# enoche/MMRec

Measured on NVIDIA H100. Metric: graph-prop edges/sec (+ full-catalog scored-items/sec in extra) @ d=64, higher is better.
Workload: dtype f32

## Files before the change

mmrec_b200/csrc/project_tc.cu:

```cuda
#include "tc_common.cuh"

namespace mmrec {

using namespace tc;

constexpr int PJ_M = 128;
constexpr int PJ_KC = 32;
constexpr int PJ_LBO_A = 2064;
constexpr int PJ_A_BYTES = (PJ_KC / 4) * PJ_LBO_A;
constexpr int PJ_CONV = 256;
constexpr int PJ_THREADS = PJ_CONV + 32;
template <int N> constexpr int pj_depth() { return N == 64 ? 3 : (N == 128 ? 2 : 1); }

struct ProjParams {
    const float* table; int64_t F; const int64_t* idx; int64_t n_out;
    const float *Whi, *Wlo;
    int N, n_chunks, chunks_per_split, n_splits, stages, vec_ok, n_tiles;
    float* partial;
    int64_t rows_padded;
};

struct PjSmem {
    uint32_t a0, b0, bars, total, stage_bytes, b_bytes;
};
__host__ __device__ inline PjSmem pj_smem(int N, int stages) {
    PjSmem L;
    L.b_bytes = (uint32_t)N * PJ_KC * 4;
    L.stage_bytes = 2 * PJ_A_BYTES + 2 * L.b_bytes;
    L.a0 = 0;
    L.b0 = 2 * PJ_A_BYTES;
    L.bars = stages * L.stage_bytes;
    L.total = L.bars + 32 * 8;
    return L;
}

template <int N, bool FAST>
__global__ void __launch_bounds__(PJ_THREADS, 1) project_tc_kernel(const ProjParams p) {
    constexpr int PJ_DEPTH = pj_depth<N>();
    extern __shared__ __align__(1024) uint8_t smem[];
    const PjSmem L = pj_smem(N, p.stages);
    const uint32_t sbase = smem_u32(smem);
    const uint32_t bar = sbase + L.bars;
    const int warp = threadIdx.x >> 5, lane = threadIdx.x & 31;
    if (threadIdx.x == 0) {
        for (int s = 0; s < 8; ++s) { mbar_init(bar + s * 8, PJ_CONV); mbar_init(bar + (8 + s) * 8, 1); mbar_init(bar + (16 + s) * 8, PJ_CONV / 32); }
        mbar_fence_init();
    }
    __syncthreads();

    const int tile = blockIdx.x / p.n_splits, sp = blockIdx.x % p.n_splits;
    const int c0 = sp * p.chunks_per_split;
    const int c1 = min(p.n_chunks, c0 + p.chunks_per_split);
    const int n_my = c1 - c0;
    const int rot = n_my > 0 ? ((int)(((int64_t)tile * n_my) / p.n_tiles) / PJ_DEPTH * PJ_DEPTH) % n_my : 0;

    if (warp == PJ_CONV / 32) {
        if (lane == 0) {
            int s = 0;
            uint32_t par = 1;
            for (int c = 0; c < n_my; ++c) {
                mbar_wait(bar + (16 + s) * 8, par);
                mbar_expect_tx(bar + (8 + s) * 8, 2 * L.b_bytes);
                const int64_t off = (int64_t)(c0 + (c + rot) % n_my) * (L.b_bytes / 4);
                bulk_g2s(sbase + s * L.stage_bytes + L.b0, p.Whi + off, L.b_bytes, bar + (8 + s) * 8);
                bulk_g2s(sbase + s * L.stage_bytes + L.b0 + L.b_bytes, p.Wlo + off, L.b_bytes, bar + (8 + s) * 8);
                if (++s == p.stages) { s = 0; par ^= 1; }
            }
        }
        return;
    }
    const int t = threadIdx.x;
    const int g = t >> 7;
    const int kb = t & 7;
    const float* rowp[4];
#pragma unroll
    for (int i = 0; i < 4; ++i) {
        const int64_t r = (int64_t)tile * PJ_M + (t >> 3) + 32 * i;
        rowp[i] = r < p.n_out ? p.table + (p.idx ? p.idx[r] : r) * p.F : nullptr;
    }
    int ld_c = rot;
    const float* kp[4];
#pragma unroll
    for (int i = 0; i < 4; ++i) kp[i] = rowp[i] ? rowp[i] + (int64_t)c0 * PJ_KC + kb * 4 : nullptr;
    auto load_chunk = [&](int c, float4 (&x)[4]) {
        if (FAST) {
            const bool on = c < n_my;
#pragma unroll
            for (int i = 0; i < 4; ++i)
                x[i] = (on && kp[i]) ? __ldg(reinterpret_cast<const float4*>(kp[i] + ld_c * PJ_KC)) : make_float4(0.f, 0.f, 0.f, 0.f);
            if (on && ++ld_c == n_my) ld_c = 0;
            return;
        }
        const int64_t k = (int64_t)(c0 + (c + rot) % n_my) * PJ_KC + kb * 4;
#pragma unroll
        for (int i = 0; i < 4; ++i) {
            float4 v = make_float4(0.f, 0.f, 0.f, 0.f);
            if (rowp[i] && c < n_my) {
                if (p.vec_ok && k + 3 < p.F) v = __ldg(reinterpret_cast<const float4*>(rowp[i] + k));
                else {
                    if (k + 0 < p.F) v.x = __ldg(rowp[i] + k + 0);
                    if (k + 1 < p.F) v.y = __ldg(rowp[i] + k + 1);
                    if (k + 2 < p.F) v.z = __ldg(rowp[i] + k + 2);
                    if (k + 3 < p.F) v.w = __ldg(rowp[i] + k + 3);
                }
            }
            x[i] = v;
        }
    };
    const uint32_t LBO_B = (uint32_t)(N / 8) * 128;
    const uint64_t a_hi0 = smem_desc(sbase + L.a0 + g * 1024, PJ_LBO_A, 128), a_lo0 = smem_desc(sbase + L.a0 + PJ_A_BYTES + g * 1024, PJ_LBO_A, 128);
    const uint64_t b_hi0 = smem_desc(sbase + L.b0, LBO_B, 128), b_lo0 = smem_desc(sbase + L.b0 + L.b_bytes, LBO_B, 128);
    const uint64_t ka = (2 * PJ_LBO_A) >> 4, kbs = (2 * LBO_B) >> 4;
    float acc[N / 2];
#pragma unroll
    for (int i = 0; i < N / 2; ++i) acc[i] = 0.f;
    uint32_t first = 0;
    int prev = 0;
    float4 ringA[PJ_DEPTH][4], ringB[PJ_DEPTH][4];
    int s = 0;
    uint32_t par = 1;
    int done = 0;
    auto fill = [&](int cbase, float4 (&ring)[PJ_DEPTH][4]) {
#pragma unroll
        for (int q = 0; q < PJ_DEPTH; ++q) load_chunk(cbase + q, ring[q]);
    };
    auto drain = [&](int cbase, float4 (&ring)[PJ_DEPTH][4]) {
#pragma unroll
        for (int q = 0; q < PJ_DEPTH; ++q) {
            if (cbase + q < n_my) {
                mbar_wait(bar + (16 + s) * 8, par);
                uint8_t* st = smem + s * L.stage_bytes;
#pragma unroll
                for (int i = 0; i < 4; ++i) {
                    const int r = (t >> 3) + 32 * i;
                    const uint32_t off = kb * PJ_LBO_A + (r >> 3) * 128 + (r & 7) * 16;
                    float4 h, l;
                    split_tf32_trunc(ring[q][i].x, h.x, l.x); split_tf32_trunc(ring[q][i].y, h.y, l.y);
                    split_tf32_trunc(ring[q][i].z, h.z, l.z); split_tf32_trunc(ring[q][i].w, h.w, l.w);
                    *reinterpret_cast<float4*>(st + L.a0 + off) = h;
                    *reinterpret_cast<float4*>(st + L.a0 + PJ_A_BYTES + off) = l;
                }
                fence_proxy_async();
                mbar_arrive(bar + s * 8);
                mbar_wait(bar + s * 8, par ^ 1);
                mbar_wait(bar + (8 + s) * 8, par ^ 1);
                const uint64_t st_off = (uint64_t)(s * L.stage_bytes) >> 4;
                uint64_t a_hi = a_hi0 + st_off, a_lo = a_lo0 + st_off, b_hi = b_hi0 + st_off, b_lo = b_lo0 + st_off;
                wgmma_fence();
#pragma unroll
                for (int j = 0; j < PJ_KC / 8; ++j) {
                    wgmma_tf32<N>(acc, a_hi, b_hi, first);
                    first = 1;
                    wgmma_tf32<N>(acc, a_lo, b_hi, 1);
                    wgmma_tf32<N>(acc, a_hi, b_lo, 1);
                    a_hi += ka; a_lo += ka; b_hi += kbs; b_lo += kbs;
                }
                wgmma_commit();
                if (done++ > 0) {
                    wgmma_wait<1>();
                    warp_arrive(bar + (16 + prev) * 8);
                }
                prev = s;
                if (++s == p.stages) { s = 0; par ^= 1; }
            }
        }
    };
    fill(0, ringA);
    for (int cb = 0; cb < n_my; cb += 2 * PJ_DEPTH) {
        fill(cb + PJ_DEPTH, ringB);
        drain(cb, ringA);
        fill(cb + 2 * PJ_DEPTH, ringA);
        drain(cb + PJ_DEPTH, ringB);
    }
    wgmma_wait<0>();
    wgmma_fence_regs(acc);
    const int w = (t >> 5) & 3;
    const int64_t row0 = (int64_t)tile * PJ_M + g * 64 + w * 16 + (lane >> 2);
#pragma unroll
    for (int h = 0; h < 2; ++h) {
        float* dst = p.partial + ((int64_t)sp * p.rows_padded + row0 + 8 * h) * N + 2 * (lane & 3);
#pragma unroll
        for (int j = 0; j < N / 8; ++j)
            *reinterpret_cast<float2*>(dst + 8 * j) = make_float2(acc[4 * j + 2 * h], acc[4 * j + 2 * h + 1]);
    }
}

__global__ void __launch_bounds__(256) project_reduce_kernel(int64_t n_out, int d, int N, int n_splits, int64_t rows_padded,
                                                             const float* __restrict__ partial, const float* __restrict__ bias,
                                                             int l2, float* __restrict__ Y, int64_t ldy) {
    const int lane = threadIdx.x & 31;
    const int64_t row = (int64_t)blockIdx.x * 8 + (threadIdx.x >> 5);
    if (row >= n_out) return;
    float acc[8];
    float ss = 0.f;
#pragma unroll
    for (int i = 0; i < 8; ++i) {
        const int c = lane + 32 * i;
        float a = 0.f;
        if (c < d) {
            for (int s = 0; s < n_splits; ++s) a += partial[((int64_t)s * rows_padded + row) * N + c];
            if (bias) a += __ldg(bias + c);
            ss += a * a;
        }
        acc[i] = a;
    }
    float inv = 1.f;
    if (l2) { ss = warp_sum(ss); inv = 1.0f / fmaxf(sqrtf(ss), 1e-12f); }
#pragma unroll
    for (int i = 0; i < 8; ++i) {
        const int c = lane + 32 * i;
        if (c < d) Y[row * ldy + c] = l2 ? acc[i] * inv : acc[i];
    }
}

struct PjPlan {
    int N, KP, n_chunks, n_splits, chunks_per_split, stages;
    int64_t n_tiles, rows_padded;
    size_t off_whi, off_wlo, off_partial, total;
};

static bool pj_plan(int64_t n_out, int64_t F, int d, PjPlan& P) {
    if (d > 256 || n_out <= 0 || F < 1) return false;
    P.N = d <= 64 ? 64 : (d <= 128 ? 128 : 256);
    P.KP = (int)((F + PJ_KC - 1) / PJ_KC * PJ_KC);
    P.n_chunks = P.KP / PJ_KC;
    P.n_tiles = (n_out + PJ_M - 1) / PJ_M;
    P.rows_padded = P.n_tiles * PJ_M;
    const int sms = sm_count();
    int splits = (int)(sms / P.n_tiles);
    if (splits < 1) splits = 1;
    if (splits > P.n_chunks / 4) splits = P.n_chunks / 4 > 0 ? P.n_chunks / 4 : 1;
    if (splits > 32) splits = 32;
    P.chunks_per_split = (P.n_chunks + splits - 1) / splits;
    P.n_splits = (P.n_chunks + P.chunks_per_split - 1) / P.chunks_per_split;
    const uint32_t stage = 2 * PJ_A_BYTES + 2 * (uint32_t)P.N * PJ_KC * 4;
    P.stages = (int)((220 * 1024) / stage);
    if (P.stages > 8) P.stages = 8;
    if (P.stages < 2) return false;
    size_t off = 0;
    auto take = [&](size_t bytes) { size_t o = off; off += align_up(bytes, 1024); return o; };
    P.off_whi = take((size_t)P.N * P.KP * 4);
    P.off_wlo = take((size_t)P.N * P.KP * 4);
    P.off_partial = take((size_t)P.n_splits * P.rows_padded * P.N * 4);
    P.total = off + 1024;
    return true;
}

size_t project_tc_workspace_bytes(int64_t n_out, int64_t F, int d) {
    PjPlan P;
    return pj_plan(n_out, F, d, P) ? P.total : 0;
}

template <int R>
static int pack_weights(const float* W, int64_t F, int d, int KP, float* hi, float* lo, cudaStream_t stream) {
    const int64_t total = (int64_t)R * (KP / 4);
    pack_split_kernel<R><<<(unsigned)((total + 255) / 256), 256, 0, stream>>>(d, nullptr, W, F, (int)F, KP, hi, lo, 1);
    MMREC_LAUNCH_CHECK();
    return MMREC_OK;
}

int project_tc(int64_t n_out, const int64_t* idx, const float* table, int64_t F, const float* W, const float* bias, int d,
               int l2_normalize, float* Y, int64_t ldy, void* ws, size_t ws_bytes, cudaStream_t stream) {
    PjPlan P;
    if (!ws || !pj_plan(n_out, F, d, P) || ws_bytes < P.total || F >= (1ll << 31)) return 0;
    char* base = (char*)(((uintptr_t)ws + 1023) & ~(uintptr_t)1023);
    float *Whi = (float*)(base + P.off_whi), *Wlo = (float*)(base + P.off_wlo), *partial = (float*)(base + P.off_partial);
    int rc = P.N == 64 ? pack_weights<64>(W, F, d, P.KP, Whi, Wlo, stream)
                       : (P.N == 128 ? pack_weights<128>(W, F, d, P.KP, Whi, Wlo, stream) : pack_weights<256>(W, F, d, P.KP, Whi, Wlo, stream));
    if (rc) return rc;
    ProjParams p;
    p.table = table; p.F = F; p.idx = idx; p.n_out = n_out; p.Whi = Whi; p.Wlo = Wlo; p.N = P.N; p.n_chunks = P.n_chunks;
    p.chunks_per_split = P.chunks_per_split; p.n_splits = P.n_splits; p.stages = P.stages;
    p.n_tiles = (int)P.n_tiles;
    p.vec_ok = ((F & 3) == 0) && ((((uintptr_t)table) & 15) == 0);
    p.partial = partial; p.rows_padded = P.rows_padded;
    const PjSmem L = pj_smem(P.N, P.stages);
    rc = set_smem_once<project_tc_kernel<64, true>, project_tc_kernel<64, false>, project_tc_kernel<128, true>,
                       project_tc_kernel<128, false>, project_tc_kernel<256, true>, project_tc_kernel<256, false>>(227 * 1024);
    if (rc) return rc;
    const bool fast = p.vec_ok && (F % PJ_KC) == 0;
    const unsigned grid = (unsigned)(P.n_tiles * P.n_splits);
    if (P.N == 64) {
        if (fast) project_tc_kernel<64, true><<<grid, PJ_THREADS, L.total, stream>>>(p);
        else project_tc_kernel<64, false><<<grid, PJ_THREADS, L.total, stream>>>(p);
    } else if (P.N == 128) {
        if (fast) project_tc_kernel<128, true><<<grid, PJ_THREADS, L.total, stream>>>(p);
        else project_tc_kernel<128, false><<<grid, PJ_THREADS, L.total, stream>>>(p);
    } else {
        if (fast) project_tc_kernel<256, true><<<grid, PJ_THREADS, L.total, stream>>>(p);
        else project_tc_kernel<256, false><<<grid, PJ_THREADS, L.total, stream>>>(p);
    }
    MMREC_LAUNCH_CHECK();
    project_reduce_kernel<<<(unsigned)((n_out + 7) / 8), 256, 0, stream>>>(n_out, d, P.N, P.n_splits, P.rows_padded, partial, bias,
                                                                         l2_normalize, Y, ldy);
    MMREC_LAUNCH_CHECK();
    return 1;
}

}
```

mmrec_b200/csrc/spmm.cu:

```cuda
#include <cooperative_groups.h>

#include "common.cuh"

namespace mmrec {

struct SpmmParams {
    int64_t n_rows, n_cols;
    const int32_t* rowptr; const int32_t* colidx; const float* vals;
    const int4* tasks; int64_t n_tasks, n_heavy; const int4* split_rows; int32_t* counters; float* partial;
    const float* X; int64_t ldx;
    float* Y; int64_t ldy;
    const float* acc_in; float* acc_out; int64_t ldacc; float acc_div;
    const float* gate_ref; int64_t ldgate;
    int y_acc;
    const float* post; int64_t post_row0; uint32_t spost;
    int d;
    uint32_t sx, sy, sacc, sgate;
    const float* X_hi; const float* acc_in_hi;
    int x_split, acc_split;
    uint32_t sx_hi, sacc_hi;
};


__device__ __forceinline__ const float4* row_f4(const float* base, uint32_t stride, int r, int f4) {
    return reinterpret_cast<const float4*>(reinterpret_cast<const char*>(base) + (uint64_t)(uint32_t)r * stride) + f4;
}
__device__ __forceinline__ float4* row_f4(float* base, uint32_t stride, int r, int f4) {
    return reinterpret_cast<float4*>(reinterpret_cast<char*>(base) + (uint64_t)(uint32_t)r * stride) + f4;
}

template <bool TWO>
__device__ __forceinline__ float4 acc_in_f4(const SpmmParams& p, int r, int f4) {
    const bool hi = TWO && r >= p.acc_split;
    return *row_f4(hi ? p.acc_in_hi : p.acc_in, hi ? p.sacc_hi : p.sacc, hi ? r - p.acc_split : r, f4);
}

template <int D, int T>
struct VecCfg {
    static_assert(D % (4 * T) == 0, "row must split into float4 per lane");
    static constexpr int V = D / (4 * T);
    static constexpr int GPW = 32 / T;
    static constexpr int UNR = (V >= 4) ? 2 : (V == 2 ? 4 : 8);
};

template <int D, int T>
__device__ __forceinline__ void spmm_epilogue(const SpmmParams& p, bool on, int row, int l, float4 (&y)[VecCfg<D, T>::V],
                                              const float4 (&accin)[VecCfg<D, T>::V]) {
    using C = VecCfg<D, T>;
    if (p.gate_ref) {
        float dot = 0.f, ny = 0.f, nr = 0.f;
        if (on) {
#pragma unroll
            for (int v = 0; v < C::V; ++v) {
                float4 r = __ldg(row_f4(p.gate_ref, p.sgate, row, v * T + l));
                dot += y[v].x * r.x + y[v].y * r.y + y[v].z * r.z + y[v].w * r.w;
                ny += y[v].x * y[v].x + y[v].y * y[v].y + y[v].z * y[v].z + y[v].w * y[v].w;
                nr += r.x * r.x + r.y * r.y + r.z * r.z + r.w * r.w;
            }
        }
#pragma unroll
        for (int o = T / 2; o > 0; o >>= 1) {
            dot += __shfl_xor_sync(0xffffffffu, dot, o);
            ny += __shfl_xor_sync(0xffffffffu, ny, o);
            nr += __shfl_xor_sync(0xffffffffu, nr, o);
        }
        float c = dot / (fmaxf(sqrtf(ny), 1e-8f) * fmaxf(sqrtf(nr), 1e-8f));
#pragma unroll
        for (int v = 0; v < C::V; ++v) { y[v].x *= c; y[v].y *= c; y[v].z *= c; y[v].w *= c; }
    }
    if (!on) return;
    if (p.Y) {
#pragma unroll
        for (int v = 0; v < C::V; ++v) {
            float4 o = y[v];
            if (p.y_acc) {
                const float4 q = *row_f4(p.Y, p.sy, row, v * T + l);
                o.x += q.x; o.y += q.y; o.z += q.z; o.w += q.w;
            }
            *row_f4(p.Y, p.sy, row, v * T + l) = o;
        }
    }
    if (p.acc_out) {
#pragma unroll
        for (int v = 0; v < C::V; ++v) {
            float4 a = y[v];
            if (p.acc_in) { a.x += accin[v].x; a.y += accin[v].y; a.z += accin[v].z; a.w += accin[v].w; }
            if (p.acc_div != 1.0f) {
                a.x = __fdiv_rn(a.x, p.acc_div); a.y = __fdiv_rn(a.y, p.acc_div);
                a.z = __fdiv_rn(a.z, p.acc_div); a.w = __fdiv_rn(a.w, p.acc_div);
            }
            if (p.post && row >= p.post_row0) {
                const float4 q = *row_f4(p.post, p.spost, row - (int)p.post_row0, v * T + l);
                a.x += q.x; a.y += q.y; a.z += q.z; a.w += q.w;
            }
            *row_f4(p.acc_out, p.sacc, row, v * T + l) = a;
        }
    }
}

template <int D, int T, bool TWO>
__device__ __forceinline__ void spmm_gather(const SpmmParams& p, int b, int len, int maxlen, int l, float4 (&acc)[VecCfg<D, T>::V]) {
    using C = VecCfg<D, T>;
    int cj[C::UNR]; float wj[C::UNR];
    const int32_t* cp = p.colidx + b;
    const float* vp = p.vals + b;
    const float* xl = p.X + l * 4;
    const float* xh = TWO ? p.X_hi + l * 4 : xl;
#pragma unroll
    for (int u = 0; u < C::UNR; ++u) {
        const bool ok = u < len;
        cj[u] = ok ? __ldg(cp + u) : 0;
        wj[u] = ok ? __ldg(vp + u) : 0.f;
    }
    for (int j0 = 0; j0 < maxlen; j0 += C::UNR, cp += C::UNR, vp += C::UNR) {
        float4 x[C::UNR][C::V];
#pragma unroll
        for (int u = 0; u < C::UNR; ++u) {
            const bool ok = j0 + u < len;
            const bool hi = TWO && cj[u] >= p.x_split;
            const float* xb = hi ? xh : xl;
            const uint32_t sb = hi ? p.sx_hi : p.sx;
            const int rb = hi ? cj[u] - p.x_split : cj[u];
#pragma unroll
            for (int v = 0; v < C::V; ++v)
                x[u][v] = ok ? __ldg(row_f4(xb, sb, rb, v * T)) : make_float4(0.f, 0.f, 0.f, 0.f);
        }
        float wc[C::UNR];
#pragma unroll
        for (int u = 0; u < C::UNR; ++u) wc[u] = wj[u];
#pragma unroll
        for (int u = 0; u < C::UNR; ++u) {
            const bool ok = j0 + C::UNR + u < len;
            cj[u] = ok ? __ldg(cp + C::UNR + u) : 0;
            wj[u] = ok ? __ldg(vp + C::UNR + u) : 0.f;
        }
#pragma unroll
        for (int u = 0; u < C::UNR; ++u) {
#pragma unroll
            for (int v = 0; v < C::V; ++v) {
                acc[v].x = fmaf(wc[u], x[u][v].x, acc[v].x);
                acc[v].y = fmaf(wc[u], x[u][v].y, acc[v].y);
                acc[v].z = fmaf(wc[u], x[u][v].z, acc[v].z);
                acc[v].w = fmaf(wc[u], x[u][v].w, acc[v].w);
            }
        }
    }
}

template <int D, int T, bool TWO>
__device__ __forceinline__ bool spmm_split_finish(const SpmmParams& p, bool split, int row, int b, int sid, int l,
                                                  float4 (&acc)[VecCfg<D, T>::V], float4 (&accin)[VecCfg<D, T>::V]) {
    using C = VecCfg<D, T>;
    int4 sr = make_int4(0, 1, 0, 1);
    int old = -1;
    bool last = false;
    if (split) {
        sr = __ldg(p.split_rows + sid);
        const int seg = (b - sr.z) / sr.w;
        float* slot = p.partial + ((int64_t)sr.x + seg) * D;
#pragma unroll
        for (int v = 0; v < C::V; ++v) *reinterpret_cast<float4*>(slot + (v * T + l) * 4) = acc[v];
        __threadfence();
    }
    __syncwarp();
    if (split && l == 0) old = atomicAdd(p.counters + sid, 1);
    old = __shfl_sync(0xffffffffu, old, 0, T);
    if (split && old == sr.y - 1) {
        __threadfence();
#pragma unroll
        for (int v = 0; v < C::V; ++v) acc[v] = make_float4(0.f, 0.f, 0.f, 0.f);
        constexpr int RB = 8;
        for (int s2 = 0; s2 < sr.y; s2 += RB) {
            float4 q[RB][C::V];
#pragma unroll
            for (int r = 0; r < RB; ++r) {
                const float* ps = p.partial + ((int64_t)sr.x + s2 + r) * D;
#pragma unroll
                for (int v = 0; v < C::V; ++v)
                    q[r][v] = (s2 + r < sr.y) ? __ldcg(reinterpret_cast<const float4*>(ps + (v * T + l) * 4))
                                              : make_float4(0.f, 0.f, 0.f, 0.f);
            }
#pragma unroll
            for (int r = 0; r < RB; ++r) {
#pragma unroll
                for (int v = 0; v < C::V; ++v) {
                    acc[v].x += q[r][v].x; acc[v].y += q[r][v].y; acc[v].z += q[r][v].z; acc[v].w += q[r][v].w;
                }
            }
        }
        if (p.acc_in) {
#pragma unroll
            for (int v = 0; v < C::V; ++v)
                accin[v] = acc_in_f4<TWO>(p, row, v * T + l);
        }
        if (l == 0) p.counters[sid] = 0;
        last = true;
    }
    __syncwarp();
    return last;
}

template <int D, int T, bool TWO>
__device__ __forceinline__ void spmm_vec_body(const SpmmParams& p, float* __restrict__ red) {
    using C = VecCfg<D, T>;
    constexpr int G = 256 / T;
    const int lane = threadIdx.x & 31, warp = threadIdx.x >> 5;
    const int g = lane / T, l = lane % T;
    const int64_t n_work = p.tasks ? p.n_tasks : p.n_rows;
    const int64_t n_heavy = p.tasks ? p.n_heavy : 0;

    for (int64_t ct = blockIdx.x; ct < n_heavy; ct += gridDim.x) {
        const int4 tk = __ldg(p.tasks + ct);
        const int row = tk.x, sid = tk.w;
        const int len = tk.z - tk.y;
        const int chunk = (len + G - 1) / G;
        const int gi = warp * C::GPW + g;
        const int mb = tk.y + gi * chunk;
        int mylen = tk.z - mb;
        mylen = mylen < 0 ? 0 : (mylen > chunk ? chunk : mylen);
        float4 accin[C::V];
#pragma unroll
        for (int v = 0; v < C::V; ++v) accin[v] = make_float4(0.f, 0.f, 0.f, 0.f);
        if (warp == 0 && g == 0 && p.acc_in && sid < 0) {
#pragma unroll
            for (int v = 0; v < C::V; ++v)
                accin[v] = acc_in_f4<TWO>(p, row, v * T + l);
        }
        float4 acc[C::V];
#pragma unroll
        for (int v = 0; v < C::V; ++v) acc[v] = make_float4(0.f, 0.f, 0.f, 0.f);
        spmm_gather<D, T, TWO>(p, mb, mylen, chunk, l, acc);
#pragma unroll
        for (int v = 0; v < C::V; ++v) *reinterpret_cast<float4*>(red + gi * D + (v * T + l) * 4) = acc[v];
        __syncthreads();
        if (warp == 0) {
#pragma unroll
            for (int v = 0; v < C::V; ++v) acc[v] = make_float4(0.f, 0.f, 0.f, 0.f);
            if (g == 0) {
                for (int q = 0; q < G; ++q) {
#pragma unroll
                    for (int v = 0; v < C::V; ++v) {
                        const float4 r4 = *reinterpret_cast<const float4*>(red + q * D + (v * T + l) * 4);
                        acc[v].x += r4.x; acc[v].y += r4.y; acc[v].z += r4.z; acc[v].w += r4.w;
                    }
                }
            }
            bool do_epi = g == 0 && sid < 0;
            if (sid >= 0) do_epi = spmm_split_finish<D, T, TWO>(p, g == 0, row, tk.y, sid, l, acc, accin);
            spmm_epilogue<D, T>(p, do_epi, row, l, acc, accin);
        }
        __syncthreads();
    }

    const int64_t W = (int64_t)gridDim.x * (blockDim.x >> 5);
    const int64_t w = (int64_t)blockIdx.x * (blockDim.x >> 5) + warp;
    const int64_t n_light = n_work - n_heavy;
    auto slot_of = [&](int64_t it) -> int64_t { return it * W + ((it & 1) ? (W - 1 - w) : w); };
    auto fetch = [&](int64_t slot) -> int4 {
        const int64_t t = slot * C::GPW + g;
        if (t >= n_light) return make_int4(-1, 0, 0, -1);
        if (p.tasks) return __ldg(p.tasks + n_heavy + t);
        return make_int4((int)t, __ldg(p.rowptr + t), __ldg(p.rowptr + t + 1), -1);
    };
    const int64_t n_slots = (n_light + C::GPW - 1) / C::GPW;
    const int64_t n_iter = (n_slots + W - 1) / W;
    int4 nxt = fetch(slot_of(0));
    for (int64_t it = 0; it < n_iter; ++it) {
        const int row = nxt.x, b = nxt.y, sid = nxt.w;
        const int len = nxt.z - nxt.y;
        const bool valid = row >= 0;
        nxt = fetch(slot_of(it + 1));
        const int maxlen = __reduce_max_sync(0xffffffffu, valid ? len : 0);
        float4 accin[C::V];
#pragma unroll
        for (int v = 0; v < C::V; ++v) accin[v] = make_float4(0.f, 0.f, 0.f, 0.f);
        if (valid && p.acc_in && sid < 0) {
#pragma unroll
            for (int v = 0; v < C::V; ++v)
                accin[v] = acc_in_f4<TWO>(p, row, v * T + l);
        }
        float4 acc[C::V];
#pragma unroll
        for (int v = 0; v < C::V; ++v) acc[v] = make_float4(0.f, 0.f, 0.f, 0.f);
        spmm_gather<D, T, TWO>(p, b, valid ? len : 0, maxlen, l, acc);
        bool do_epi = valid && sid < 0;
        const bool split = valid && sid >= 0;
        if (__any_sync(0xffffffffu, split)) {
            if (spmm_split_finish<D, T, TWO>(p, split, row, b, sid, l, acc, accin)) do_epi = true;
        }
        spmm_epilogue<D, T>(p, do_epi, row, l, acc, accin);
    }
}

template <int D, int T>
__global__ void __launch_bounds__(256) spmm_vec_kernel(const SpmmParams p) {
    __shared__ __align__(16) float red[(256 / T) * D];
    spmm_vec_body<D, T, false>(p, red);
}

constexpr int SPMM_CHAIN_MAX = 8;
struct SpmmChain { SpmmParams step[SPMM_CHAIN_MAX]; int n; unsigned sync_mask; };

template <int D, int T, bool COOP>
__global__ void __launch_bounds__(256, 3) spmm_chain_kernel(const SpmmChain c) {
    __shared__ __align__(16) float red[(256 / T) * D];
    for (int i = 0; i < c.n; ++i) {
        if (COOP && ((c.sync_mask >> i) & 1u)) { __threadfence(); cooperative_groups::this_grid().sync(); }
        spmm_vec_body<D, T, true>(c.step[i], red);
    }
}

__global__ void __launch_bounds__(256) spmm_generic_kernel(const SpmmParams p) {
    const int lane = threadIdx.x & 31;
    const int64_t warp0 = (int64_t)blockIdx.x * (blockDim.x >> 5) + (threadIdx.x >> 5);
    const int64_t nwarps = (int64_t)gridDim.x * (blockDim.x >> 5);
    for (int64_t row = warp0; row < p.n_rows; row += nwarps) {
        const int b = p.rowptr[row], e = p.rowptr[row + 1];
        float dot = 0.f, ny = 0.f, nr = 0.f;
        if (p.gate_ref) {
            for (int k0 = 0; k0 < p.d; k0 += 32) {
                const int k = k0 + lane;
                float acc = 0.f;
                if (k < p.d)
                    for (int j = b; j < e; ++j) acc = fmaf(p.vals[j], p.X[(int64_t)p.colidx[j] * p.ldx + k], acc);
                float r = k < p.d ? p.gate_ref[row * p.ldgate + k] : 0.f;
                dot += acc * r; ny += acc * acc; nr += r * r;
            }
            dot = warp_sum(dot); ny = warp_sum(ny); nr = warp_sum(nr);
        }
        const float c = p.gate_ref ? dot / (fmaxf(sqrtf(ny), 1e-8f) * fmaxf(sqrtf(nr), 1e-8f)) : 1.f;
        for (int k0 = 0; k0 < p.d; k0 += 32) {
            const int k = k0 + lane;
            if (k >= p.d) continue;
            float acc = 0.f;
            for (int j = b; j < e; ++j) acc = fmaf(p.vals[j], p.X[(int64_t)p.colidx[j] * p.ldx + k], acc);
            if (p.gate_ref) acc *= c;
            if (p.Y) p.Y[row * p.ldy + k] = p.y_acc ? p.Y[row * p.ldy + k] + acc : acc;
            if (p.acc_out) {
                float a = acc + (p.acc_in ? p.acc_in[row * p.ldacc + k] : 0.f);
                if (p.acc_div != 1.0f) a = __fdiv_rn(a, p.acc_div);
                if (p.post && row >= p.post_row0) a += p.post[(row - p.post_row0) * (int64_t)(p.spost / 4) + k];
                p.acc_out[row * p.ldacc + k] = a;
            }
        }
    }
}

static thread_local int g_spmm_y_acc = 0;
int g_spmm_lanes = 0;

template <int D, int T>
static int launch_vec(const SpmmParams& p, cudaStream_t stream) {
    static int blocks_per_sm = 0;
    if (!blocks_per_sm) {
        MMREC_CUDA(cudaOccupancyMaxActiveBlocksPerMultiprocessor(&blocks_per_sm, spmm_vec_kernel<D, T>, 256, 0));
        if (blocks_per_sm < 1) blocks_per_sm = 1;
    }
    const int64_t n_work = p.tasks ? p.n_tasks : p.n_rows;
    const int per_block = 8 * (32 / T);
    int64_t grid = (n_work - p.n_heavy + per_block - 1) / per_block;
    if (grid < p.n_heavy) grid = p.n_heavy;
    const int64_t cap = (int64_t)sm_count() * blocks_per_sm;
    if (grid > cap) grid = cap;
    if (grid < 1) return MMREC_OK;
    spmm_vec_kernel<D, T><<<(unsigned)grid, 256, 0, stream>>>(p);
    MMREC_LAUNCH_CHECK();
    return MMREC_OK;
}

template <int D>
static int launch_vec_d(const SpmmParams& p, cudaStream_t stream) {
    constexpr int T4 = D / 4 > 32 ? 32 : D / 4;
    constexpr int T8 = D / 8 > 32 ? 32 : D / 8;
    constexpr int T16 = D / 16 > 32 ? 32 : D / 16;
    int T = g_spmm_lanes ? g_spmm_lanes : T4;
    if (T == T4) return launch_vec<D, T4>(p, stream);
    if (T == T16) return launch_vec<D, T16>(p, stream);
    return launch_vec<D, T8>(p, stream);
}

}

using namespace mmrec;

extern "C" int mmrec_spmm_set_lanes(int lanes_per_row) {
    MMREC_CHECK_ARG(lanes_per_row == 0 || lanes_per_row == 2 || lanes_per_row == 4 || lanes_per_row == 8 ||
                    lanes_per_row == 16 || lanes_per_row == 32, "spmm_set_lanes: 0 (default) or a power of two <= 32");
    g_spmm_lanes = lanes_per_row;
    return MMREC_OK;
}

extern "C" int mmrec_spmm_f32(int64_t n_rows, int64_t n_cols, int d, const int32_t* rowptr, const int32_t* colidx,
                              const float* vals, const int32_t* tasks, int64_t n_tasks, int64_t n_cta_tasks,
                              const int32_t* split_rows,
                              int32_t* counters, float* partial, const float* X, int64_t ldx, float* Y, int64_t ldy,
                              const float* acc_in, float* acc_out, int64_t ldacc, float acc_div, const float* gate_ref,
                              int64_t ldgate, void* stream_) {
    cudaStream_t stream = (cudaStream_t)stream_;
    MMREC_CHECK_ARG(n_rows >= 0 && n_cols >= 0 && d >= 1, "spmm: bad sizes");
    if (n_rows == 0) return MMREC_OK;
    MMREC_CHECK_ARG(rowptr && X && (Y || acc_out), "spmm: null pointer");
    MMREC_CHECK_ARG(ldx >= d && (!Y || ldy >= d) && (!acc_out || ldacc >= d) && (!gate_ref || ldgate >= d), "spmm: leading dimension < d");
    MMREC_CHECK_ARG(acc_div != 0.0f, "spmm: acc_div == 0");
    MMREC_CHECK_ARG(!tasks || (n_tasks >= 0 && n_cta_tasks >= 0 && n_cta_tasks <= n_tasks && split_rows && counters && partial),
                    "spmm: plan pointers missing");
    SpmmParams p;
    p.n_rows = n_rows; p.n_cols = n_cols; p.rowptr = rowptr; p.colidx = colidx; p.vals = vals;
    p.tasks = (const int4*)tasks; p.n_tasks = n_tasks; p.n_heavy = tasks ? n_cta_tasks : 0; p.split_rows = (const int4*)split_rows;
    p.counters = counters; p.partial = partial; p.X = X; p.ldx = ldx; p.Y = Y; p.ldy = ldy;
    p.acc_in = acc_in; p.acc_out = acc_out; p.ldacc = ldacc; p.acc_div = acc_div; p.gate_ref = gate_ref;
    p.ldgate = ldgate; p.d = d;
    p.post = nullptr; p.post_row0 = 0; p.spost = 0; p.y_acc = g_spmm_y_acc;
    MMREC_CHECK_ARG(!(p.y_acc && gate_ref), "spmm: y_accumulate does not combine with the cosine gate");
    MMREC_CHECK_ARG(ldx < (1ll << 30) && ldy < (1ll << 30) && ldacc < (1ll << 30) && ldgate < (1ll << 30) && n_cols < (1ll << 31) &&
                    n_rows < (1ll << 31), "spmm: leading dimension / size out of range");
    p.sx = (uint32_t)(ldx * 4); p.sy = (uint32_t)(ldy * 4); p.sacc = (uint32_t)(ldacc * 4); p.sgate = (uint32_t)(ldgate * 4);
    p.X_hi = X; p.x_split = (int)n_cols; p.sx_hi = p.sx; p.acc_in_hi = acc_in; p.acc_split = (int)n_rows; p.sacc_hi = p.sacc;
    auto al16 = [](const void* q, int64_t ld) { return q == nullptr || ((((uintptr_t)q) & 15) == 0 && (ld & 3) == 0); };
    const bool vec_ok = al16(X, ldx) && al16(Y, ldy) && al16(acc_in, ldacc) && al16(acc_out, ldacc) &&
                        al16(gate_ref, ldgate) && al16(partial, 4);
    if (vec_ok) {
        switch (d) {
            case 32: return launch_vec_d<32>(p, stream);
            case 64: return launch_vec_d<64>(p, stream);
            case 128: return launch_vec_d<128>(p, stream);
            case 256: return launch_vec_d<256>(p, stream);
            default: break;
        }
    }
    p.tasks = nullptr;
    int64_t grid = (n_rows + 7) / 8;
    const int64_t cap = (int64_t)sm_count() * 8;
    if (grid > cap) grid = cap;
    spmm_generic_kernel<<<(unsigned)grid, 256, 0, stream>>>(p);
    MMREC_LAUNCH_CHECK();
    return MMREC_OK;
}

extern "C" int mmrec_spmm_acc_f32(int64_t n_rows, int64_t n_cols, int d, const int32_t* rowptr, const int32_t* colidx,
                                  const float* vals, const int32_t* tasks, int64_t n_tasks, int64_t n_cta_tasks,
                                  const int32_t* split_rows, int32_t* counters, float* partial, const float* X, int64_t ldx, float* Y,
                                  int64_t ldy, const float* acc_in, float* acc_out, int64_t ldacc, float acc_div, int y_accumulate,
                                  void* stream_) {
    g_spmm_y_acc = y_accumulate ? 1 : 0;
    const int rc = mmrec_spmm_f32(n_rows, n_cols, d, rowptr, colidx, vals, tasks, n_tasks, n_cta_tasks, split_rows, counters, partial, X, ldx,
                                  Y, ldy, acc_in, acc_out, ldacc, acc_div, nullptr, 0, stream_);
    g_spmm_y_acc = 0;
    return rc;
}

namespace mmrec {
template <int D, bool COOP>
static int launch_chain(const SpmmChain& c, cudaStream_t stream) {
    constexpr int T = D / 4 > 32 ? 32 : D / 4;
    static int blocks_per_sm = 0;
    if (!blocks_per_sm) {
        MMREC_CUDA(cudaOccupancyMaxActiveBlocksPerMultiprocessor(&blocks_per_sm, spmm_chain_kernel<D, T, COOP>, 256, 0));
// ... 107 lines not shown
```

mmrec_b200/csrc/tc_common.cuh:

```cuda
#pragma once
#include <cuda_fp16.h>

#include "common.cuh"
#include "wgmma.cuh"

namespace mmrec {
namespace tc {

__device__ __forceinline__ uint32_t smem_u32(const void* p) { return (uint32_t)__cvta_generic_to_shared(p); }

__device__ __forceinline__ void mbar_init(uint32_t bar, uint32_t count) {
    asm volatile("mbarrier.init.shared::cta.b64 [%0], %1;" ::"r"(bar), "r"(count) : "memory");
}
__device__ __forceinline__ void mbar_fence_init() { asm volatile("fence.mbarrier_init.release.cluster;" ::: "memory"); }
__device__ __forceinline__ void mbar_arrive(uint32_t bar) {
    asm volatile("mbarrier.arrive.shared::cta.b64 _, [%0];" ::"r"(bar) : "memory");
}
__device__ __forceinline__ void mbar_expect_tx(uint32_t bar, uint32_t bytes) {
    asm volatile("mbarrier.arrive.expect_tx.shared::cta.b64 _, [%0], %1;" ::"r"(bar), "r"(bytes) : "memory");
}
__device__ __forceinline__ bool mbar_try_wait(uint32_t bar, uint32_t parity) {
    uint32_t ok;
    asm volatile(
        "{\n\t.reg .pred p;\n\t"
        "mbarrier.try_wait.parity.shared::cta.b64 p, [%1], %2;\n\t"
        "selp.u32 %0, 1, 0, p;\n\t}"
        : "=r"(ok) : "r"(bar), "r"(parity) : "memory");
    return ok != 0;
}
__device__ __forceinline__ uint64_t global_ns() {
    uint64_t t;
    asm volatile("mov.u64 %0, %%globaltimer;" : "=l"(t));
    return t;
}
__device__ __forceinline__ void mbar_wait(uint32_t bar, uint32_t parity) {
    uint32_t spins = 0;
    uint64_t t0 = 0;
    while (!mbar_try_wait(bar, parity)) {
        if (++spins == 4096u) t0 = global_ns();
        if (spins > 4096u && (spins & 1023u) == 0 && global_ns() - t0 > 2000000000ull) __trap();
    }
}

__device__ __forceinline__ void bulk_g2s(uint32_t dst_smem, const void* src, uint32_t bytes, uint32_t bar) {
    asm volatile("cp.async.bulk.shared::cluster.global.mbarrier::complete_tx::bytes [%0], [%1], %2, [%3];"
                 ::"r"(dst_smem), "l"(src), "r"(bytes), "r"(bar) : "memory");
}

__device__ __forceinline__ void wgmma_fence() { asm volatile("wgmma.fence.sync.aligned;" ::: "memory"); }
__device__ __forceinline__ void wgmma_commit() { asm volatile("wgmma.commit_group.sync.aligned;" ::: "memory"); }
template <int N>
__device__ __forceinline__ void wgmma_wait() { asm volatile("wgmma.wait_group.sync.aligned %0;" ::"n"(N) : "memory"); }
template <int R>
__device__ __forceinline__ void wgmma_fence_regs(float (&d)[R]) {
#pragma unroll
    for (int i = 0; i < R; ++i) asm volatile("" : "+f"(d[i])::"memory");
}
__device__ __forceinline__ void fence_proxy_async() { asm volatile("fence.proxy.async.shared::cta;" ::: "memory"); }
__device__ __forceinline__ void warp_arrive(uint32_t bar) {
    __syncwarp();
    if ((threadIdx.x & 31) == 0) mbar_arrive(bar);
}

__device__ __forceinline__ uint64_t smem_desc(uint32_t smem_addr, uint32_t lbo_bytes, uint32_t sbo_bytes) {
    uint64_t d = 0;
    d |= (uint64_t)((smem_addr & 0x3FFFFu) >> 4);
    d |= (uint64_t)((lbo_bytes >> 4) & 0x3FFFu) << 16;
    d |= (uint64_t)((sbo_bytes >> 4) & 0x3FFFu) << 32;
    return d;
}

__device__ __forceinline__ void split_tf32(float x, float& hi, float& lo) {
    uint32_t h, l;
    asm("cvt.rna.tf32.f32 %0, %1;" : "=r"(h) : "f"(x));
    hi = __uint_as_float(h);
    asm("cvt.rna.tf32.f32 %0, %1;" : "=r"(l) : "f"(x - hi));
    lo = __uint_as_float(l);
}

__device__ __forceinline__ void split_tf32_trunc(float x, float& hi, float& lo) {
    hi = __uint_as_float(__float_as_uint(x) & 0xffffe000u);
    lo = x - hi;
}

}

__device__ __forceinline__ float fp16_scale_for(uint32_t m_bits) {
    const uint32_t e = (m_bits >> 23) & 0xffu;
    if (e == 0u || e == 255u || e < 14u) return 1.0f;
    return __uint_as_float((268u - e) << 23);
}

__global__ void absmax_norm_kernel(int64_t n, const float* __restrict__ X, int64_t ldx, int F, float* __restrict__ rnorm,
                                   uint32_t* __restrict__ amax, uint32_t* __restrict__ nmax);

__device__ __forceinline__ void store_fp16x8(uint4* __restrict__ out, int64_t tile, int kblks, int kb, int rr, const float (&x)[8], float sc) {
    uint32_t w[4];
#pragma unroll
    for (int e = 0; e < 4; ++e) {
        const __half2 h = __floats2half2_rn(x[2 * e] * sc, x[2 * e + 1] * sc);
        w[e] = *reinterpret_cast<const uint32_t*>(&h);
    }
    out[((tile * kblks + kb) * 16 + rr / 8) * 8 + (rr % 8)] = make_uint4(w[0], w[1], w[2], w[3]);
}

template <int GPT, class Dst>
__device__ __forceinline__ void group_max_store(const float (&acc)[64], int e2, int q, int n_valid, int64_t row, int64_t n_rows, Dst dst) {
    auto val = [&](int j, int e) { return 8 * j + 2 * q + e < n_valid ? acc[4 * j + 2 * e2 + e] : -INFINITY; };
    float gm[GPT];
#pragma unroll
    for (int g = 0; g < GPT; ++g) {
        float m = -INFINITY;
#pragma unroll
        for (int j = g * (16 / GPT); j < (g + 1) * (16 / GPT); ++j) m = fmaxf(m, fmaxf(val(j, 0), val(j, 1)));
        m = fmaxf(m, __shfl_xor_sync(0xffffffffu, m, 1));
        gm[g] = fmaxf(m, __shfl_xor_sync(0xffffffffu, m, 2));
    }
    if (row < n_rows) {
        float* d = dst();
#pragma unroll
        for (int g = 0; g < GPT; ++g)
            if ((g & 3) == q) d[g] = gm[g];
    }
}

__device__ __forceinline__ void set_threshold(float t, float margin, float* thr, int32_t* flag) {
    const bool finite = fabsf(t) < INFINITY && margin < INFINITY;
    *thr = finite ? t - margin : INFINITY;
    *flag = finite ? 0 : 2;
}

constexpr int TC_M = 128;
constexpr int TC_N = 256;
constexpr int TC_KC = 32;
constexpr int TC_SLAB_BYTES = TC_N * TC_KC * 4;
constexpr int TC_THREADS = 288;

template <int R>
__device__ __forceinline__ void pack_split_one(int64_t t, int64_t n_rows, const int64_t* __restrict__ idx, const float* __restrict__ E,
                                               int64_t ld, int d, int KP, float* __restrict__ hi, float* __restrict__ lo) {
    const int kblks = KP / 4;
    const int64_t row = t / kblks;
    const int kb = (int)(t % kblks);
    float x[4] = {0.f, 0.f, 0.f, 0.f};
    if (row < n_rows) {
        const float* src = E + (idx ? idx[row] : row) * ld;
#pragma unroll
        for (int e = 0; e < 4; ++e)
            if (kb * 4 + e < d) x[e] = __ldg(src + kb * 4 + e);
    }
    float4 h, l;
    tc::split_tf32(x[0], h.x, l.x); tc::split_tf32(x[1], h.y, l.y); tc::split_tf32(x[2], h.z, l.z); tc::split_tf32(x[3], h.w, l.w);
    const int64_t tile = row / R;
    const int rr = (int)(row % R);
    const int64_t off = ((tile * kblks + kb) * (R / 8) + rr / 8) * 32 + (rr % 8) * 4;
    *reinterpret_cast<float4*>(hi + off) = h;
    *reinterpret_cast<float4*>(lo + off) = l;
}

template <int R>
__global__ void pack_split_kernel(int64_t n_rows, const int64_t* __restrict__ idx, const float* __restrict__ E, int64_t ld,
                                  int d, int KP, float* __restrict__ hi, float* __restrict__ lo, int64_t n_tiles) {
    const int64_t t = blockIdx.x * (int64_t)blockDim.x + threadIdx.x;
    if (t >= n_tiles * R * (KP / 4)) return;
    pack_split_one<R>(t, n_rows, idx, E, ld, d, KP, hi, lo);
}

}
```

Measured before the change: 13.76 billion.

## Add TMA-fed projection kernel with in-smem tf32 split and tune SpMM launch bounds

Adds a warp-specialized projection kernel that loads the dense feature table through a 2D TMA tensor map with 128B swizzle. The consumer warpgroups split each tile into tf32 hi/lo parts in shared memory, replacing the converter-thread gather path whenever no index array is given. Separately, SpMM vec and chain kernels get per-config minimum-CTA launch bounds, and the unroll factor for the narrowest rows drops from 8 to 4. The weight packing kernel is also remapped so consecutive threads cover different rows. The new projection path relies on driver entry-point lookup and adds a shared-memory lo ring plus named barriers per chunk.

After: 15.07 billion (median of 6 runs). +9.5%, better.

```diff
diff --git a/mmrec_b200/csrc/project_tc.cu b/mmrec_b200/csrc/project_tc.cu
--- a/mmrec_b200/csrc/project_tc.cu
+++ b/mmrec_b200/csrc/project_tc.cu
@@ -1,3 +1,5 @@
+#include <cudaTypedefs.h>
+
 #include "tc_common.cuh"
 
 namespace mmrec {
@@ -171,6 +173,145 @@
         drain(cb, ringA);
         fill(cb + 2 * PJ_DEPTH, ringA);
         drain(cb + PJ_DEPTH, ringB);
+    }
+    wgmma_wait<0>();
+    wgmma_fence_regs(acc);
+    const int w = (t >> 5) & 3;
+    const int64_t row0 = (int64_t)tile * PJ_M + g * 64 + w * 16 + (lane >> 2);
+#pragma unroll
+    for (int h = 0; h < 2; ++h) {
+        float* dst = p.partial + ((int64_t)sp * p.rows_padded + row0 + 8 * h) * N + 2 * (lane & 3);
+#pragma unroll
+        for (int j = 0; j < N / 8; ++j)
+            *reinterpret_cast<float2*>(dst + 8 * j) = make_float2(acc[4 * j + 2 * h], acc[4 * j + 2 * h + 1]);
+    }
+}
+
+constexpr int PT_HALF_BYTES = 64 * PJ_KC * 4;
+constexpr int PT_TILE_BYTES = 2 * PT_HALF_BYTES;
+constexpr int PT_SMEM_LIMIT = 227 * 1024;
+
+struct PtSmem {
+    uint32_t lo0, b0, stage_bytes, b_bytes, bars, total;
+};
+__host__ __device__ inline PtSmem pt_smem(int N, int stages) {
+    PtSmem L;
+    L.b_bytes = (uint32_t)N * PJ_KC * 4;
+    L.stage_bytes = PT_TILE_BYTES + 2 * L.b_bytes;
+    L.b0 = PT_TILE_BYTES;
+    L.lo0 = stages * L.stage_bytes;
+    L.bars = L.lo0 + 2 * PT_TILE_BYTES;
+    L.total = L.bars + 32 * 8 + 1024;
+    return L;
+}
+__host__ __device__ inline int pt_stages(int N) {
+    const int fixed = 2 * PT_TILE_BYTES + 32 * 8 + 1024;
+    const int s = (PT_SMEM_LIMIT - fixed) / (PT_TILE_BYTES + 2 * N * PJ_KC * 4);
+    return s > 8 ? 8 : s;
+}
+
+template <int N>
+__global__ void __launch_bounds__(PJ_THREADS, 1) project_tma_kernel(const __grid_constant__ CUtensorMap tmap, const ProjParams p) {
+    extern __shared__ uint8_t smem_raw[];
+    const PtSmem L = pt_smem(N, p.stages);
+    const uint32_t sbase = (smem_u32(smem_raw) + 1023u) & ~1023u;
+    uint8_t* smem = smem_raw + (sbase - smem_u32(smem_raw));
+    const uint32_t bar = sbase + L.bars;
+    auto b_full = [&](int s) { return bar + s * 8; };
+    auto a_full = [&](int s, int g) { return bar + (8 + 2 * s + g) * 8; };
+    auto empty = [&](int s) { return bar + (24 + s) * 8; };
+    const int warp = threadIdx.x >> 5, lane = threadIdx.x & 31;
+    if (threadIdx.x == 0) {
+        for (int s = 0; s < p.stages; ++s) {
+            mbar_init(b_full(s), 1); mbar_init(a_full(s, 0), 1); mbar_init(a_full(s, 1), 1); mbar_init(empty(s), PJ_CONV / 32);
+        }
+        mbar_fence_init();
+    }
+    __syncthreads();
+
+    const int tile = blockIdx.x / p.n_splits, sp = blockIdx.x % p.n_splits;
+    const int c0 = sp * p.chunks_per_split;
+    const int c1 = min(p.n_chunks, c0 + p.chunks_per_split);
+    const int n_my = c1 - c0;
+    constexpr int ROT = pj_depth<N>();
+    const int rot = n_my > 0 ? ((int)(((int64_t)tile * n_my) / p.n_tiles) / ROT * ROT) % n_my : 0;
+
+    if (warp == PJ_CONV / 32) {
+        if (lane == 0) {
+            const int row0 = tile * PJ_M;
+            const bool half1 = row0 + 64 < p.n_out;
+            int s = 0;
+            uint32_t par = 1;
+            for (int c = 0; c < n_my; ++c) {
+                mbar_wait(empty(s), par);
+                const int ck = c0 + (c + rot) % n_my;
+                const int64_t off = (int64_t)ck * (L.b_bytes / 4);
+                const uint32_t st = sbase + s * L.stage_bytes;
+                mbar_expect_tx(b_full(s), 2 * L.b_bytes);
+                bulk_g2s(st + L.b0, p.Whi + off, L.b_bytes, b_full(s));
+                bulk_g2s(st + L.b0 + L.b_bytes, p.Wlo + off, L.b_bytes, b_full(s));
+                mbar_expect_tx(a_full(s, 0), PT_HALF_BYTES);
+                tma_load_2d(st, &tmap, ck * PJ_KC, row0, a_full(s, 0));
+                if (half1) {
+                    mbar_expect_tx(a_full(s, 1), PT_HALF_BYTES);
+                    tma_load_2d(st + PT_HALF_BYTES, &tmap, ck * PJ_KC, row0 + 64, a_full(s, 1));
+                } else {
+                    mbar_arrive(a_full(s, 1));
+                }
+                if (++s == p.stages) { s = 0; par ^= 1; }
+            }
+        }
+        return;
+    }
+    const int t = threadIdx.x;
+    const int g = t >> 7, tg = t & 127;
+    const uint32_t LBO_B = (uint32_t)(N / 8) * 128;
+    const uint64_t a_hi0 = smem_desc_sw128(sbase + g * PT_HALF_BYTES);
+    const uint64_t lo_slot = (uint64_t)PT_TILE_BYTES >> 4;
+    const uint64_t a_lo0 = smem_desc_sw128(sbase + L.lo0 + g * PT_HALF_BYTES);
+    const uint64_t b_hi0 = smem_desc(sbase + L.b0, LBO_B, 128), b_lo0 = smem_desc(sbase + L.b0 + L.b_bytes, LBO_B, 128);
+    const uint64_t ka = 32 >> 4, kbs = (2 * LBO_B) >> 4;
+    float acc[N / 2];
+#pragma unroll
+    for (int i = 0; i < N / 2; ++i) acc[i] = 0.f;
+    uint32_t first = 0;
+    int prev = 0, s = 0;
+    uint32_t ph = 0;
+    for (int c = 0; c < n_my; ++c) {
+        mbar_wait(a_full(s, g), ph);
+        uint8_t* a = smem + s * L.stage_bytes + g * PT_HALF_BYTES;
+        uint8_t* lo = smem + L.lo0 + (c & 1) * PT_TILE_BYTES + g * PT_HALF_BYTES;
+#pragma unroll
+        for (int i = 0; i < 4; ++i) {
+            const uint32_t off = (uint32_t)(tg + 128 * i) * 16;
+            const float4 x = *reinterpret_cast<const float4*>(a + off);
+            float4 h, l;
+            split_tf32_trunc(x.x, h.x, l.x); split_tf32_trunc(x.y, h.y, l.y);
+            split_tf32_trunc(x.z, h.z, l.z); split_tf32_trunc(x.w, h.w, l.w);
+            *reinterpret_cast<float4*>(a + off) = h;
+            *reinterpret_cast<float4*>(lo + off) = l;
+        }
+        fence_proxy_async();
+        named_bar_sync(1 + g, 128);
+        mbar_wait(b_full(s), ph);
+        const uint64_t st_off = (uint64_t)(s * L.stage_bytes) >> 4;
+        uint64_t a_hi = a_hi0 + st_off, a_lo = a_lo0 + (c & 1) * lo_slot, b_hi = b_hi0 + st_off, b_lo = b_lo0 + st_off;
+        wgmma_fence();
+#pragma unroll
+        for (int j = 0; j < PJ_KC / 8; ++j) {
+            wgmma_tf32<N>(acc, a_hi, b_hi, first);
+            first = 1;
+            wgmma_tf32<N>(acc, a_lo, b_hi, 1);
+            wgmma_tf32<N>(acc, a_hi, b_lo, 1);
+            a_hi += ka; a_lo += ka; b_hi += kbs; b_lo += kbs;
+        }
+        wgmma_commit();
+        if (c > 0) {
+            wgmma_wait<1>();
+            warp_arrive(empty(prev));
+        }
+        prev = s;
+        if (++s == p.stages) { s = 0; ph ^= 1; }
     }
     wgmma_wait<0>();
     wgmma_fence_regs(acc);
@@ -252,10 +393,43 @@
 }
 
 template <int R>
+__global__ void pj_pack_weights_kernel(int d, const float* __restrict__ W, int64_t F, int KP, float* __restrict__ hi,
+                                       float* __restrict__ lo) {
+    const int64_t t = blockIdx.x * (int64_t)blockDim.x + threadIdx.x;
+    if (t >= (int64_t)R * (KP / 4)) return;
+    pack_split_one<R>((t % R) * (KP / 4) + t / R, d, nullptr, W, F, (int)F, KP, hi, lo);
+}
+
+template <int R>
 static int pack_weights(const float* W, int64_t F, int d, int KP, float* hi, float* lo, cudaStream_t stream) {
     const int64_t total = (int64_t)R * (KP / 4);
-    pack_split_kernel<R><<<(unsigned)((total + 255) / 256), 256, 0, stream>>>(d, nullptr, W, F, (int)F, KP, hi, lo, 1);
+    pj_pack_weights_kernel<R><<<(unsigned)((total + 255) / 256), 256, 0, stream>>>(d, W, F, KP, hi, lo);
     MMREC_LAUNCH_CHECK();
+    return MMREC_OK;
+}
+
+static int pt_tensor_map(const float* table, int64_t n_out, int64_t F, CUtensorMap* map) {
+    static PFN_cuTensorMapEncodeTiled_v12000 encode = [] {
+        void* fn = nullptr;
+        cudaDriverEntryPointQueryResult q;
+        if (cudaGetDriverEntryPoint("cuTensorMapEncodeTiled", &fn, cudaEnableDefault, &q) != cudaSuccess || q != cudaDriverEntryPointSuccess)
+            fn = nullptr;
+        return reinterpret_cast<PFN_cuTensorMapEncodeTiled_v12000>(fn);
+    }();
+    if (!encode) {
+        set_error("project: the driver has no cuTensorMapEncodeTiled");
+        return MMREC_ECUDA;
+    }
+    const cuuint64_t dims[2] = {(cuuint64_t)F, (cuuint64_t)n_out};
+    const cuuint64_t strides[1] = {(cuuint64_t)F * 4};
+    const cuuint32_t box[2] = {PJ_KC, 64}, estr[2] = {1, 1};
+    const CUresult r = encode(map, CU_TENSOR_MAP_DATA_TYPE_FLOAT32, 2, const_cast<float*>(table), dims, strides, box, estr,
+                              CU_TENSOR_MAP_INTERLEAVE_NONE, CU_TENSOR_MAP_SWIZZLE_128B, CU_TENSOR_MAP_L2_PROMOTION_L2_256B,
+                              CU_TENSOR_MAP_FLOAT_OOB_FILL_NONE);
+    if (r != CUDA_SUCCESS) {
+        set_error("project: cuTensorMapEncodeTiled failed (%d) for a [%lld, %lld] table", (int)r, (long long)n_out, (long long)F);
+        return MMREC_ECUDA;
+    }
     return MMREC_OK;
 }
 
@@ -274,12 +448,29 @@
     p.n_tiles = (int)P.n_tiles;
     p.vec_ok = ((F & 3) == 0) && ((((uintptr_t)table) & 15) == 0);
     p.partial = partial; p.rows_padded = P.rows_padded;
+    const unsigned grid = (unsigned)(P.n_tiles * P.n_splits);
+    if (!idx && p.vec_ok) {
+        CUtensorMap map;
+        rc = pt_tensor_map(table, n_out, F, &map);
+        if (rc) return rc;
+        rc = set_smem_once<project_tma_kernel<64>, project_tma_kernel<128>, project_tma_kernel<256>>(PT_SMEM_LIMIT);
+        if (rc) return rc;
+        p.stages = pt_stages(P.N);
+        const uint32_t smem = pt_smem(P.N, p.stages).total;
+        if (P.N == 64) project_tma_kernel<64><<<grid, PJ_THREADS, smem, stream>>>(map, p);
+        else if (P.N == 128) project_tma_kernel<128><<<grid, PJ_THREADS, smem, stream>>>(map, p);
+        else project_tma_kernel<256><<<grid, PJ_THREADS, smem, stream>>>(map, p);
+        MMREC_LAUNCH_CHECK();
+        project_reduce_kernel<<<(unsigned)((n_out + 7) / 8), 256, 0, stream>>>(n_out, d, P.N, P.n_splits, P.rows_padded, partial,
+                                                                             bias, l2_normalize, Y, ldy);
+        MMREC_LAUNCH_CHECK();
+        return 1;
+    }
     const PjSmem L = pj_smem(P.N, P.stages);
     rc = set_smem_once<project_tc_kernel<64, true>, project_tc_kernel<64, false>, project_tc_kernel<128, true>,
                        project_tc_kernel<128, false>, project_tc_kernel<256, true>, project_tc_kernel<256, false>>(227 * 1024);
     if (rc) return rc;
     const bool fast = p.vec_ok && (F % PJ_KC) == 0;
-    const unsigned grid = (unsigned)(P.n_tiles * P.n_splits);
     if (P.N == 64) {
         if (fast) project_tc_kernel<64, true><<<grid, PJ_THREADS, L.total, stream>>>(p);
         else project_tc_kernel<64, false><<<grid, PJ_THREADS, L.total, stream>>>(p);
diff --git a/mmrec_b200/csrc/spmm.cu b/mmrec_b200/csrc/spmm.cu
--- a/mmrec_b200/csrc/spmm.cu
+++ b/mmrec_b200/csrc/spmm.cu
@@ -40,7 +40,9 @@
     static_assert(D % (4 * T) == 0, "row must split into float4 per lane");
     static constexpr int V = D / (4 * T);
     static constexpr int GPW = 32 / T;
-    static constexpr int UNR = (V >= 4) ? 2 : (V == 2 ? 4 : 8);
+    static constexpr int UNR = (V >= 4) ? 2 : 4;
+    static constexpr int MIN_CTAS_VEC = V == 1 ? 4 : 1;
+    static constexpr int MIN_CTAS_CHAIN = V == 1 ? 4 : 3;
 };
 
 template <int D, int T>
@@ -293,7 +295,7 @@
 }
 
 template <int D, int T>
-__global__ void __launch_bounds__(256) spmm_vec_kernel(const SpmmParams p) {
+__global__ void __launch_bounds__(256, (VecCfg<D, T>::MIN_CTAS_VEC)) spmm_vec_kernel(const SpmmParams p) {
     __shared__ __align__(16) float red[(256 / T) * D];
     spmm_vec_body<D, T, false>(p, red);
 }
@@ -302,7 +304,7 @@
 struct SpmmChain { SpmmParams step[SPMM_CHAIN_MAX]; int n; unsigned sync_mask; };
 
 template <int D, int T, bool COOP>
-__global__ void __launch_bounds__(256, 3) spmm_chain_kernel(const SpmmChain c) {
+__global__ void __launch_bounds__(256, (VecCfg<D, T>::MIN_CTAS_CHAIN)) spmm_chain_kernel(const SpmmChain c) {
     __shared__ __align__(16) float red[(256 / T) * D];
     for (int i = 0; i < c.n; ++i) {
         if (COOP && ((c.sync_mask >> i) & 1u)) { __threadfence(); cooperative_groups::this_grid().sync(); }
diff --git a/mmrec_b200/csrc/tc_common.cuh b/mmrec_b200/csrc/tc_common.cuh
--- a/mmrec_b200/csrc/tc_common.cuh
+++ b/mmrec_b200/csrc/tc_common.cuh
@@ -46,6 +46,13 @@
     asm volatile("cp.async.bulk.shared::cluster.global.mbarrier::complete_tx::bytes [%0], [%1], %2, [%3];"
                  ::"r"(dst_smem), "l"(src), "r"(bytes), "r"(bar) : "memory");
 }
+__device__ __forceinline__ void tma_load_2d(uint32_t dst_smem, const void* tmap, int x, int y, uint32_t bar) {
+    asm volatile("cp.async.bulk.tensor.2d.shared::cluster.global.tile.mbarrier::complete_tx::bytes [%0], [%1, {%2, %3}], [%4];"
+                 ::"r"(dst_smem), "l"(tmap), "r"(x), "r"(y), "r"(bar) : "memory");
+}
+__device__ __forceinline__ void named_bar_sync(uint32_t id, uint32_t count) {
+    asm volatile("bar.sync %0, %1;" ::"r"(id), "r"(count) : "memory");
+}
 
 __device__ __forceinline__ void wgmma_fence() { asm volatile("wgmma.fence.sync.aligned;" ::: "memory"); }
 __device__ __forceinline__ void wgmma_commit() { asm volatile("wgmma.commit_group.sync.aligned;" ::: "memory"); }
@@ -68,6 +75,9 @@
     d |= (uint64_t)((lbo_bytes >> 4) & 0x3FFFu) << 16;
     d |= (uint64_t)((sbo_bytes >> 4) & 0x3FFFu) << 32;
     return d;
+}
+__device__ __forceinline__ uint64_t smem_desc_sw128(uint32_t smem_addr) {
+    return smem_desc(smem_addr, 16, 1024) | (1ull << 62);
 }
 
 __device__ __forceinline__ void split_tf32(float x, float& hi, float& lo) {
```
